# CERALIVE/ceracoder

Hardware: AMD Instinct MI355X
Metric: 1080p H.264 encoded frames/sec per GPU (higher is better)
Workload: dtype u8

## Files before the change

### ceracoder_amd/csrc/k_motion.hip

```cpp
#include "kernels_common.hpp"

#ifndef ME_MBS
#define ME_MBS 4
#endif
#define ME_WQ (ME_MBS + 2)
#define ME_ROWS 50
#define ME_STRIDE 53
#define ME_K 5

DEV unsigned long long qsad(unsigned lo, unsigned hi, unsigned cur, unsigned long long acc) {
    unsigned long long src = ((unsigned long long)hi << 32) | lo;
    return __builtin_amdgcn_qsad_pk_u16_u8(src, cur, acc);
}
DEV int mv_bits(int v) {
    int a = iabs(v);
    return a == 0 ? 1 : 7 + 2 * (31 - __clz(a));
}
DEV int med3(int a, int b, int c) {
    const int lo = a < b ? a : b, hi = a < b ? b : a;
    return c < lo ? lo : (c > hi ? hi : c);
}
struct fpred_t { int px, py, sx, sy; };
DEV fpred_t field_pred(const imv_t *__restrict__ f, int mbw, int mx, int my, bool top) {
    const bool avA = mx > 0, avB = top, avC = top && mx + 1 < mbw, avD = mx > 0 && top, hasC = avC || avD;
// ... 220 lines not shown
#pragma unroll
        for (int d = 0; d < ME_K; d++) { const uint2 v = ldg64(sf + (ME_K * g + d) * SURF_COLS); acc[d] = ((unsigned long long)v.y << 32) | v.x; }
        const unsigned best = select_min(acc, g, dxg, active, ctx->me_range, ctx->lambda, jpx, jpy, jsx, jsy);
        if (lane == 0) store_imv(&out[mbn], best, ctx->lambda, jpx, jpy, jsx, jsy);
    }
}

#define SP_GS 24
#define SP_PS 20
struct sp_lds {
    uint8_t G[23 * SP_GS];
    int16_t H1[18 * SP_GS];
    uint8_t b[19 * SP_PS];
    uint8_t h[18 * SP_GS];
    uint8_t j[18 * SP_PS];
    uint8_t pad[16];
};
typedef short sp_s2 __attribute__((ext_vector_type(2)));
DEV sp_s2 as_s2(unsigned v) { return __builtin_bit_cast(sp_s2, v); }
DEV unsigned as_u(sp_s2 v) { return __builtin_bit_cast(unsigned, v); }
DEV sp_s2 bytes_lo(unsigned w) { return as_s2(__builtin_amdgcn_perm(0u, w, 0x0c010c00u)); }
DEV sp_s2 bytes_hi(unsigned w) { return as_s2(__builtin_amdgcn_perm(0u, w, 0x0c030c02u)); }
DEV sp_s2 clip255_s2(sp_s2 v) { return __builtin_elementwise_min(__builtin_elementwise_max(v, (sp_s2)(0)), (sp_s2)(255)); }
DEV sp_s2 pair_s2(int a, int b) { return as_s2(__builtin_amdgcn_perm((unsigned)b, (unsigned)a, 0x05040100u)); }
DEV unsigned pack_s2(sp_s2 lo, sp_s2 hi) { return __builtin_amdgcn_perm(as_u(hi), as_u(lo), 0x06040200u); }
DEV unsigned clip_pack4(int a, int b, int c, int d) { return pack_s2(clip255_s2(pair_s2(a, b)), clip255_s2(pair_s2(c, d))); }
DEV int mvq_bits(int q) {
    unsigned k = q > 0 ? (unsigned)(2 * q - 1) : (unsigned)(-2 * q);
    return 2 * (31 - __clz((int)(k + 1))) + 1;
}
DEV unsigned lds4(const uint8_t *plane, int o) {
    const unsigned *w = (const unsigned *)(plane + (o & ~3));
    return __builtin_amdgcn_alignbyte(w[1], w[0], (unsigned)(o & 3));
}
DEV unsigned sp_sample4(const sp_lds *L, int X, int Y, int fx, int fy) {
#define SG(x, y) lds4(L->G, ((y) + 2) * SP_GS + (x) + 2)
#define SB(x, y) lds4(L->b, (y) * SP_PS + (x))
#define SH(x, y) lds4(L->h, (y) * SP_GS + (x) + 2)
#define SJ(x, y) lds4(L->j, (y) * SP_PS + (x))
    if (fy == 0) {
        if (fx == 0) return SG(X, Y);
        return fx == 2 ? SB(X, Y) : fx == 1 ? avg4(SG(X, Y), SB(X, Y)) : avg4(SG(X + 1, Y), SB(X, Y));
    }
    if (fx == 0) return fy == 2 ? SH(X, Y) : fy == 1 ? avg4(SG(X, Y), SH(X, Y)) : avg4(SG(X, Y + 1), SH(X, Y));
    if ((fx & 1) && (fy & 1)) return avg4(fy == 1 ? SB(X, Y) : SB(X, Y + 1), fx == 1 ? SH(X, Y) : SH(X + 1, Y));
    if (fx == 2 && fy == 2) return SJ(X, Y);
    if (fx == 2) return avg4(fy == 1 ? SB(X, Y) : SB(X, Y + 1), SJ(X, Y));
    return avg4(fx == 1 ? SH(X, Y) : SH(X + 1, Y), SJ(X, Y));
#undef SG
#undef SB
#undef SH
#undef SJ
}
DEV void sp_planes(sp_lds *L, const int lane) {
    if (lane < 54) {
        const int d = lane % 6, seg = lane / 6;
        sp_s2 lo[7], hi[7];
#pragma unroll
        for (int r = 0; r < 7; r++) {
            const unsigned w = *(const unsigned *)&L->G[(2 * seg + r) * SP_GS + 4 * d];
            lo[r] = bytes_lo(w); hi[r] = bytes_hi(w);
        }
#pragma unroll
        for (int t = 0; t < 2; t++) {
            const sp_s2 vl = (lo[t + 2] + lo[t + 3]) * (sp_s2)(20) - (lo[t + 1] + lo[t + 4]) * (sp_s2)(5) + (lo[t] + lo[t + 5]);
            const sp_s2 vh = (hi[t + 2] + hi[t + 3]) * (sp_s2)(20) - (hi[t + 1] + hi[t + 4]) * (sp_s2)(5) + (hi[t] + hi[t + 5]);
            const int R = 2 * seg + t;
            unsigned *o = (unsigned *)&L->H1[R * SP_GS + 4 * d];
            o[0] = as_u(vl); o[1] = as_u(vh);
            *(unsigned *)&L->h[R * SP_GS + 4 * d] = pack_s2(clip255_s2((vl + (sp_s2)(16)) >> (sp_s2)(5)), clip255_s2((vh + (sp_s2)(16)) >> (sp_s2)(5)));
        }
    }
#pragma unroll
    for (int it = 0; it < 2; it++) {
        const int i = lane + 64 * it;
        if (i < 19 * 5) {
            const int R = i / 5, g = i - R * 5;
            const unsigned *gw = (const unsigned *)&L->G[(R + 2) * SP_GS + 4 * g];
            const unsigned d0 = gw[0] ^ 0x80808080u, d1 = gw[1] ^ 0x80808080u, d2 = gw[2] ^ 0x80808080u;
            int o[4];
#pragma unroll
            for (int k = 0; k < 4; k++) {
                const unsigned w0 = k ? __builtin_amdgcn_alignbyte(d1, d0, (unsigned)k) : d0, w1 = k ? __builtin_amdgcn_alignbyte(d2, d1, (unsigned)k) : d1;
                const int v = __builtin_amdgcn_sdot4((int)w0, 0x1414FB01, __builtin_amdgcn_sdot4((int)w1, 0x000001FB, 4096, false), false);
                o[k] = (v + 16) >> 5;
            }
            *(unsigned *)&L->b[R * SP_PS + 4 * g] = clip_pack4(o[0], o[1], o[2], o[3]);
        }
    }
    WAVE_SYNC();
#pragma unroll
    for (int it = 0; it < 2; it++) {
        const int i = lane + 64 * it;
        if (i < 18 * 5) {
            const int R = i / 5, g = i - R * 5;
            const unsigned *hw = (const unsigned *)&L->H1[R * SP_GS + 4 * g];
            const unsigned p0 = hw[0], p1 = hw[1], p2 = hw[2], p3 = hw[3], p4 = hw[4];
            const unsigned q0 = __builtin_amdgcn_alignbyte(p1, p0, 2u), q1 = __builtin_amdgcn_alignbyte(p2, p1, 2u),
                           q2 = __builtin_amdgcn_alignbyte(p3, p2, 2u), q3 = __builtin_amdgcn_alignbyte(p4, p3, 2u);
            const sp_s2 ca = {1, -5}, cb = {20, 20}, cc = {-5, 1};
#define J3(a, b, c) __builtin_amdgcn_sdot2(as_s2(a), ca, __builtin_amdgcn_sdot2(as_s2(b), cb, __builtin_amdgcn_sdot2(as_s2(c), cc, 512, false), false), false)
            const int v0 = J3(p0, p1, p2), v1 = J3(q0, q1, q2), v2 = J3(p1, p2, p3), v3 = J3(q1, q2, q3);
#undef J3
            *(unsigned *)&L->j[R * SP_PS + 4 * g] = clip_pack4(v0 >> 10, v1 >> 10, v2 >> 10, v3 >> 10);
        }
    }
// ... 27 lines not shown
            L->G[r * SP_GS + c] = (uint8_t)ldg8(ref + (size_t)yy * stride + xx);
        }
    const int pr = lane >> 2, pc = (lane & 3) * 4;
    unsigned curw;
    {
        int sy = y0 + pr;
        sy = sy < ctx->vis_h ? sy : ctx->vis_h - 1;
        curw = ldg32(ctx->src_y + (size_t)sy * ctx->src_stride + x0 + pc);
    }
    WAVE_SYNC();
    sp_planes(L, lane);
    const int lambda = ctx->lambda;
    int bqx = info.mvx, bqy = info.mvy;
    unsigned best = info.cost;
#pragma unroll 1
    for (int step = 2; step >= 1; step--) {
        const int cqx = bqx, cqy = bqy;
        unsigned acc[4] = {0, 0, 0, 0};
#pragma unroll
        for (int c8 = 0; c8 < 8; c8++) {
            const int k = c8 < 4 ? c8 : c8 + 1;
            const int qx = cqx + (k % 3 - 1) * step, qy = cqy + (k / 3 - 1) * step;
            const int ox = qx - info.mvx, oy = qy - info.mvy;
            const int X = 1 + (ox >> 2) + pc, Y = 1 + (oy >> 2) + pr;
            const unsigned sad = __builtin_amdgcn_sad_u8(curw, sp_sample4(L, X, Y, ox & 3, oy & 3), 0u);
            acc[c8 >> 1] |= sad << (16 * (c8 & 1));
        }
#pragma unroll
        for (int q = 0; q < 4; q++) {
            acc[q] = (unsigned)wave64_sum((int)acc[q]);
        }
#pragma unroll
        for (int c8 = 0; c8 < 8; c8++) {
            const int k = c8 < 4 ? c8 : c8 + 1;
            const int qx = cqx + (k % 3 - 1) * step, qy = cqy + (k / 3 - 1) * step;
            const unsigned sad = (acc[c8 >> 1] >> (16 * (c8 & 1))) & 0xFFFFu;
            const unsigned cost = sad + (unsigned)(lambda * (mvq_bits(qx) + mvq_bits(qy)));
            if (cost < best) { best = cost; bqx = qx; bqy = qy; }
        }
    }
    if (lane == 0 && ok) {
        mb_info_t *mb = &ctx->mbi[mbn];
        stg32(&mb->mvx, ((unsigned)(uint16_t)bqx) | ((unsigned)(uint16_t)bqy << 16));
        stg32(&mb->cost, best);
    }
}

DEV int dec_score(unsigned M) { return dec_score_mask(M); }
DEV int row_or4(int v) {
    v |= __builtin_amdgcn_update_dpp(0, v, 0x128, 0xF, 0xF, false);
    v |= __builtin_amdgcn_update_dpp(0, v, 0x124, 0xF, 0xF, false);
    return v;
}
DEV unsigned ref_word4(const uint8_t *__restrict__ ref, int stride, int W, int H, int x, int y, bool inside) {
    if (inside) {
        const uint8_t *b = ref + (size_t)y * stride + (x & ~3);
        return __builtin_amdgcn_alignbyte(ldg32(b + 4), ldg32(b), (unsigned)(x & 3));
    }
    const uint8_t *r = ref + (size_t)clip3(0, H - 1, y) * stride;
    return pack4((int)ldg8(r + clip3(0, W - 1, x)), (int)ldg8(r + clip3(0, W - 1, x + 1)), (int)ldg8(r + clip3(0, W - 1, x + 2)), (int)ldg8(r + clip3(0, W - 1, x + 3)));
}
DEV void chroma_pred4(const frame_ctx_t *__restrict__ ctx, int lane, int x0, int y0, int W, int H, int mvx, int mvy, int *pd) {
    const int stride = ctx->stride;
    const int py = (lane >> 2) & 3, cby = (lane >> 4) & 1, c = (lane >> 1) & 1, cbx = lane & 1;
    const int cx0 = x0 >> 1, cy0 = y0 >> 1, cw = W >> 1, ch = H >> 1;
    const int cy = cby * 4 + py, cxb = cbx * 4;
    const int xi = mvx >> 3, yi = mvy >> 3, xf = mvx & 7, yf = mvy & 7;
    const uint8_t *__restrict__ rf = ctx->ref_uv;
    int A[5], B[5];
    if (cx0 + xi >= 0 && cx0 + xi + 9 <= cw && cy0 + yi >= 0 && cy0 + yi + 9 <= ch) {
        const int o = 2 * (cx0 + cxb + xi) + c, a = o & 3;
        const uint8_t *r0 = rf + (size_t)(cy0 + cy + yi) * stride + (o & ~3), *r1 = r0 + stride;
        const unsigned a0 = ldg32(r0), a1 = ldg32(r0 + 4), a2 = ldg32(r0 + 8), b0 = ldg32(r1), b1 = ldg32(r1 + 4), b2 = ldg32(r1 + 8);
        const unsigned sa0 = __builtin_amdgcn_alignbyte(a1, a0, (unsigned)a), sa1 = __builtin_amdgcn_alignbyte(a2, a1, (unsigned)a);
        const unsigned sb0 = __builtin_amdgcn_alignbyte(b1, b0, (unsigned)a), sb1 = __builtin_amdgcn_alignbyte(b2, b1, (unsigned)a);
        A[0] = byte_of(sa0, 0); A[1] = byte_of(sa0, 2); A[2] = byte_of(sa1, 0); A[3] = byte_of(sa1, 2); A[4] = (int)((a2 >> (8 * a)) & 255);
        B[0] = byte_of(sb0, 0); B[1] = byte_of(sb0, 2); B[2] = byte_of(sb1, 0); B[3] = byte_of(sb1, 2); B[4] = (int)((b2 >> (8 * a)) & 255);
    } else {
        const int ya = clip3(0, ch - 1, cy0 + cy + yi), yb = clip3(0, ch - 1, cy0 + cy + yi + 1);
#pragma unroll
        for (int i = 0; i < 5; i++) {
            const int xx = clip3(0, cw - 1, cx0 + cxb + i + xi);
            A[i] = (int)ldg8(rf + (size_t)ya * stride + 2 * xx + c);
            B[i] = (int)ldg8(rf + (size_t)yb * stride + 2 * xx + c);
        }
    }
    const int w00 = (8 - xf) * (8 - yf), w10 = xf * (8 - yf), w01 = (8 - xf) * yf, w11 = xf * yf;
#pragma unroll
    for (int i = 0; i < 4; i++) pd[i] = (w00 * A[i] + w10 * A[i + 1] + w01 * B[i] + w11 * B[i + 1] + 32) >> 6;
}
DEV unsigned pmb_luma_tq(const dev_tables *T, int lane, unsigned curw, unsigned pw, int qp, bool decimate, int *lev, int *x) {
    const int py = (lane >> 2) & 3, fy = ((py & 1) << 1) | (py >> 1);
    const col_bf cb = make_col_bf(py);
    const int kz0 = (int)((0xFEA9DB83C7426510ull >> (16 * fy)) & 0xFFFF);
    const qparams q = make_q(T, qp, false);
    const int mfe = py < 2 ? q.mf[0] : q.mf[2], mfo = py < 2 ? q.mf[2] : q.mf[1], ve = py < 2 ? q.v[0] : q.v[2], vo = py < 2 ? q.v[2] : q.v[1];
#pragma unroll
    for (int i = 0; i < 4; i++) x[i] = byte_of(curw, i) - byte_of(pw, i);
    fwd_rows4(x);
    unsigned m = 0, big = 0;
#pragma unroll
    for (int i = 0; i < 4; i++) {
        const int cf = fwd_col(x[i], cb);
        lev[i] = quant1(cf, (i & 1) ? mfo : mfe, q.f, q.qbits);
        m |= (lev[i] != 0 ? 1u : 0u) << ((kz0 >> (4 * i)) & 15);
        big |= (lev[i] > 1 || lev[i] < -1) ? 1u : 0u;
    }
    if (decimate) {
        const unsigned mm = (unsigned)row_or4((int)(m | (big << 16)));
        int s = (mm >> 16) ? 9 : dec_score(((mm & 0xFFFFu) << 1) | 1u);
        int s8 = s + quad_xor<1>(s);
        s8 += __shfl_xor(s8, 16, 64);
        int tot = s8 + quad_xor<2>(s8);
        tot += __shfl_xor(tot, 32, 64);
        if (s8 < 4 || tot < 6) { lev[0] = lev[1] = lev[2] = lev[3] = 0; }
    }
#pragma unroll
    for (int i = 0; i < 4; i++) x[i] = (lev[i] * ((i & 1) ? vo : ve)) << q.shift;
    const unsigned long long bal = __ballot((lev[0] | lev[1] | lev[2] | lev[3]) != 0);
    const unsigned long long t = bal | (bal >> 4) | (bal >> 8) | (bal >> 12);
    const int rb = lane & 15, rbx = blkx(rb) >> 2, rby = blky(rb) >> 2;
    return (unsigned)(__ballot(lane < 16 && ((t >> (16 * rby + rbx)) & 1)) & 0xFFFFull);
}
DEV unsigned pmb_satd(int lane, unsigned curw, unsigned pw) {
    const int py = (lane >> 2) & 3, s1 = py < 2 ? 1 : -1, s2 = (py & 1) ? -1 : 1;
    const int d0 = byte_of(curw, 0) - byte_of(pw, 0), d1 = byte_of(curw, 1) - byte_of(pw, 1), d2 = byte_of(curw, 2) - byte_of(pw, 2), d3 = byte_of(curw, 3) - byte_of(pw, 3);
    const int a = d0 + d3, b = d1 + d2, c = d1 - d2, e = d0 - d3;
    int t[4] = {a + b, e + c, a - b, e - c};
    int acc = 0;
#pragma unroll
    for (int i = 0; i < 4; i++) {
        const int u = mad24(t[i], s1, row_xor8(t[i]));
        const int w = mad24(u, s2, row_xor4(u));
        acc += iabs(w);
    }
    return (unsigned)wave64_sum(acc);
}
DEV unsigned pmb_sa8d(int lane, unsigned curw, unsigned pw) {
    const int s0 = (lane & 1) ? -1 : 1, s1 = (lane & 4) ? -1 : 1, s2 = (lane & 8) ? -1 : 1, s3 = (lane & 16) ? -1 : 1;
    const int d0 = byte_of(curw, 0) - byte_of(pw, 0), d1 = byte_of(curw, 1) - byte_of(pw, 1), d2 = byte_of(curw, 2) - byte_of(pw, 2), d3 = byte_of(curw, 3) - byte_of(pw, 3);
    const int a = d0 + d3, b = d1 + d2, c = d1 - d2, e = d0 - d3;
    int t[4] = {a + b, e + c, a - b, e - c};
    int acc = 0;
#pragma unroll
    for (int i = 0; i < 4; i++) {
        int u = mad24(t[i], s0, quad_xor<1>(t[i]));
        u = mad24(u, s1, row_xor4(u));
        u = mad24(u, s2, row_xor8(u));
        u = mad24(u, s3, __shfl_xor(u, 16, 64));
        acc += iabs(u);
    }
    return (unsigned)wave64_sum(acc);
}
DEV bool pmb_pick_t8(int lane, unsigned curw, unsigned pw) {
    const unsigned raw4 = pmb_satd(lane, curw, pw), raw8 = pmb_sa8d(lane, curw, pw);
    return __builtin_amdgcn_readfirstlane((int)(((raw8 + 2) >> 2) < (raw4 >> 1))) != 0;
}
template <bool SC1>
DEV void pmb_store_pred_only(const frame_ctx_t *__restrict__ ctx, int16_t *lv, int lane, int x0, int y0, unsigned pw, const int *pd) {
    const int stride = ctx->stride, pr = lane >> 2, pc = (lane & 3) * 4;
    stx32<SC1>(ctx->rec_y + (size_t)(y0 + pr) * stride + x0 + pc, pw);
    const int py = (lane >> 2) & 3, cby = (lane >> 4) & 1, c = (lane >> 1) & 1, cbx = lane & 1;
    const unsigned mine = pack4(pd[0], pd[1], pd[2], pd[3]), other = (unsigned)quad_xor<2>((int)mine);
    if (lane < 32 && c == 0) {
        uint2 out;
        out.x = __builtin_amdgcn_perm(other, mine, 0x05010400u);
        out.y = __builtin_amdgcn_perm(other, mine, 0x07030602u);
        stx64<SC1>(ctx->rec_uv + (size_t)((y0 >> 1) + cby * 4 + py) * stride + 2 * ((x0 >> 1) + cbx * 4), out);
    }
    if (lane < MB_LEVELS * 2 / 16) stg128(lv + 8 * lane, make_uint4(0, 0, 0, 0));
}

template <bool SC1>
DEV unsigned pmb_luma_t8(const frame_ctx_t *__restrict__ ctx, int *tile, int lane, unsigned curw, unsigned pw, int qp, int mbn, int x0, int y0) {
    const int pr = lane >> 2, pc = (lane & 3) * 4;
    {
        int *t = tile + ((pr >> 3) * 2 + (pc >> 3)) * 64 + (pr & 7) * 8 + (pc & 7);
#pragma unroll
        for (int i = 0; i < 4; i++) t[i] = byte_of(curw, i) - byte_of(pw, i);
    }
    WAVE_SYNC();
    const bool act = lane < 16;
    const int i8 = (lane >> 2) & 3, j = lane & 3;
    int *tb = tile + i8 * 64;
    const int m6 = qp % 6, k6 = qp / 6;
    int rs[2][8], cw[2][8];
    unsigned submask = 0;
    if (act) {
#pragma unroll
        for (int r = 0; r < 2; r++) {
// ... 81 lines not shown
        for (int i = 0; i < 4; i++) o[i] = clip255(byte_of(pw, i) + t[i]);
        stx32<SC1>(ctx->rec_y + (size_t)(y0 + pr) * ctx->stride + x0 + pc, pack4(o[0], o[1], o[2], o[3]));
    }
    return (unsigned)(__ballot(act && ((submask >> j) & 1u)) & 0xFFFFull);
}
DEV unsigned part_gsum(unsigned v) {
    v += (unsigned)quad_xor<1>((int)v);
    v += (unsigned)row_xor4((int)v);
    v += (unsigned)row_xor8((int)v);
    v += (unsigned)__shfl_xor((int)v, 16, 64);
    return v;
}
DEV unsigned part_total(unsigned g) { g += (unsigned)quad_xor<2>((int)g); return g + (unsigned)__shfl_xor((int)g, 32, 64); }
#ifdef PMB_PROF
#define PMB_NPH 11
#define PMB_MARK(k) do { const unsigned long long t1_ = __builtin_readcyclecounter(); ph_[k] = t1_ - t0_; t0_ = t1_; } while (0)
#define PMB_MARK0() unsigned long long ph_[PMB_NPH] = {0, 0, 0, 0, 0, 0, 0, 0, 0, 0, 0}; unsigned long long t0_ = __builtin_readcyclecounter()
#define PMB_FLUSH() do { if (lane == 0) for (int k_ = 0; k_ < PMB_NPH; k_++) stg32((unsigned *)ctx->dbrec + (size_t)mbn * 16 + k_, (unsigned)ph_[k_]); } while (0)
#else
#define PMB_MARK(k) ((void)0)
#define PMB_MARK0() ((void)0)
#define PMB_FLUSH() ((void)0)
#endif
struct pmb_pre_t { uint2 selfw; fpred_t fp; unsigned curw; uint2 sw; unsigned ds; uint4 dw; };
DEV pmb_pre_t pmb_preload(const frame_ctx_t *__restrict__ ctx, const int mbn, const int lane) {
    const int mbw = ctx->mbw, my = mbn / mbw, mx = mbn - my * mbw, x0 = mx * 16, y0 = my * 16;
    pmb_pre_t p;
    const imv_t *__restrict__ field = k_final_imv_dev(ctx);
    p.selfw = ldg64(field + mbn);
    {
        int sy = y0 + (lane >> 2);
        sy = sy < ctx->vis_h ? sy : ctx->vis_h - 1;
        p.curw = ldg32(ctx->src_y + (size_t)sy * ctx->src_stride + x0 + (lane & 3) * 4);
    }
    {
        const int cby = (lane >> 4) & 1, cbx = lane & 1;
        int sy = (y0 >> 1) + cby * 4 + ((lane >> 2) & 3);
        const int vh2 = ctx->vis_h >> 1;
        sy = sy < vh2 ? sy : vh2 - 1;
        p.sw = ldg64(ctx->src_uv + (size_t)sy * ctx->src_stride + 2 * ((x0 >> 1) + cbx * 4));
    }
    p.dw = ctx->intra_p ? ldg128(ctx->idec + (size_t)mbn * IDEC_BYTES + 16) : make_uint4(0, 0, 0, 0);
    p.fp = field_pred(field, mbw, mx, my, row_has_top(ctx, my));
    p.ds = (unsigned)*(const GAS uint16_t *)(ctx->surf + (size_t)mbn * SURF_U16 + ((p.fp.sy >> 2) + 16) * SURF_COLS + (p.fp.sx >> 2) + 16);
    return p;
}
DEV bool ir_ok(const frame_ctx_t *__restrict__ ctx, int mx, int mvx) {
    return mx >= ctx->ir_c0 || (16 * mx + 15 + (mvx >> 2) + ((mvx & 3) ? 3 : 0) <= ctx->ir_clean && 8 * mx + 7 + (mvx >> 3) + ((mvx & 7) ? 1 : 0) <= (ctx->ir_clean >> 1));
}
DEV int ir_max_whole(const frame_ctx_t *__restrict__ ctx, int mx) {
    const int kl = ctx->ir_clean - 16 * mx - 15, kc = 2 * ((ctx->ir_clean >> 1) - 8 * mx - 7);
    return 4 * (kl < kc ? kl : kc);
}
template <bool SC1>
DEV void pmb_store_intra(mb_info_t *mb, const uint4 dw, int qp, int lane) {
    if (lane == 0) {
        const bool i4 = ((dw.x >> 16) & 255u) != 0;
        mb_info_t m;
        m.mvx = 0; m.mvy = 0; m.mb_type = i4 ? 2 : 0; m.i16_mode = i4 ? 0 : (uint8_t)(dw.x & 255u); m.chroma_mode = (uint8_t)((dw.x >> 8) & 255u);
        m.qp = (uint8_t)qp; m.nzmask = 0; m.cost = dw.y;
        st_mbinfo_x<SC1>(mb, m);
    }
}
template <bool SC1, bool PART, int T8, bool IR>
DEV void pmb_mb(const frame_ctx_t *__restrict__ ctx, sp_lds *L, const int mbn, const int lane, const int refine, const pmb_pre_t &pre) {
    const int mbw = ctx->mbw, mbh = ctx->mbh, stride = ctx->stride, W = mbw * 16, H = mbh * 16, qp = mb_qp_dev(ctx, mbn), lambda = ctx->lambda;
    const int my = mbn / mbw, mx = mbn - my * mbw, x0 = mx * 16, y0 = my * 16;
    const dev_tables *T = &g_tab;
    PMB_MARK0();
    const uint2 selfw = pre.selfw;
    int imx = (int)(int16_t)(selfw.x & 0xFFFF);
    const int imy = (int)(int16_t)(selfw.x >> 16);
    const unsigned di = selfw.y & 0xFFFFu, ibits = selfw.y >> 16;
    const fpred_t fp = pre.fp;
    const int pr = lane >> 2, pc = (lane & 3) * 4;
    const int py = (lane >> 2) & 3;
    const unsigned curw = pre.curw;
    int sv[4];
    {
        const int c = (lane >> 1) & 1;
        const uint2 sw = pre.sw;
        const unsigned slo = c ? (sw.x >> 8) : sw.x, shi = c ? (sw.y >> 8) : sw.y;
        sv[0] = (int)(slo & 255); sv[1] = (int)((slo >> 16) & 255); sv[2] = (int)(shi & 255); sv[3] = (int)((shi >> 16) & 255);
    }
    int16_t *lv = ctx->levels + (size_t)mbn * MB_LEVELS;
    mb_info_t *mb = &ctx->mbi[mbn];
    if (IR && mx >= ctx->ir_c0 && mx < ctx->ir_c1) {
        pmb_store_intra<SC1>(mb, pre.dw, qp, lane);
        PMB_FLUSH();
        return;
    }
    {
        const unsigned ds = pre.ds;
        const bool skip_ok = !IR || ir_ok(ctx, mx, fp.sx);
        bool pass = ctx->drop_sad && ds < ctx->drop_sad && skip_ok;
        const bool worth = ds <= di + (unsigned)(lambda * SKIP_MARGIN_BITS) && skip_ok;
        PMB_MARK(0);
        if (pass || worth) {
            const int X = x0 + (fp.sx >> 2), Y = y0 + (fp.sy >> 2);
            const bool inside = X >= 0 && Y >= 0 && X + 16 <= W && Y + 16 <= H;
            const unsigned pw = ref_word4(ctx->ref_y, stride, W, H, X + pc, Y + pr, inside);
            int pd[4];
            chroma_pred4(ctx, lane, x0, y0, W, H, fp.sx, fp.sy, pd);
            if (!pass) {
                int lev[4], x[4];
                if (pmb_luma_tq(T, lane, curw, pw, qp, true, lev, x) == 0) {
                    unsigned nz_c = 0, dc_c = 0;
                    chroma_rows4(ctx, T, lv, x0 >> 1, y0 >> 1, lane, pd, sv, qp, false, false, nullptr, nz_c, dc_c, true, 0, SC1);
                    pass = (nz_c | dc_c) == 0;
                }
            }
            PMB_MARK(1);
            if (pass) {
                pmb_store_pred_only<SC1>(ctx, lv, lane, x0, y0, pw, pd);
                if (lane == 0) {
                    mb_info_t m;
                    m.mvx = (int16_t)fp.sx; m.mvy = (int16_t)fp.sy; m.mb_type = 1; m.i16_mode = 0; m.chroma_mode = 0; m.qp = (uint8_t)qp; m.nzmask = 0; m.cost = di;
                    st_mbinfo_x<SC1>(mb, m);
                }
                PMB_FLUSH();
                return;
            }
        }
    }
    if (IR && !ir_ok(ctx, mx, imx)) imx = ir_max_whole(ctx, mx);
    const int ix = x0 + (imx >> 2), iy = y0 + (imy >> 2);
    const uint8_t *__restrict__ ref = ctx->ref_y;
    if (ix - 3 >= 0 && iy - 3 >= 0 && ((ix - 3) & ~3) + 28 <= W && iy + 19 < H) {
        const int a = (ix - 3) & 3;
        const uint8_t *base = ref + (size_t)(iy - 3) * stride + ((ix - 3) & ~3);
        for (int i = lane; i < 23 * 6; i += 64) {
            const int r = i / 6, d = i - r * 6;
            const unsigned w0 = ldg32(base + (size_t)r * stride + 4 * d), w1 = ldg32(base + (size_t)r * stride + 4 * d + 4);
            *(unsigned *)&L->G[r * SP_GS + 4 * d] = __builtin_amdgcn_alignbyte(w1, w0, (unsigned)a);
        }
    } else
        for (int i = lane; i < 23 * 23; i += 64) {
            int r = i / 23, c = i - r * 23;
            int yy = clip3(0, H - 1, iy - 3 + r), xx = clip3(0, W - 1, ix - 3 + c);
            L->G[r * SP_GS + c] = (uint8_t)ldg8(ref + (size_t)yy * stride + xx);
        }
    WAVE_SYNC();
    PMB_MARK(2);
    int bqx = imx, bqy = imy;
    unsigned q0 = 0, qh[4] = {0, 0, 0, 0}, qq[4] = {0, 0, 0, 0};
    int hbx = imx, hby = imy;
    unsigned best;
    if (PART) {
        q0 = part_gsum(__builtin_amdgcn_sad_u8(curw, sp_sample4(L, 1 + pc, 1 + pr, 0, 0), 0u));
        best = part_total(q0) + (unsigned)(lambda * (mvq_bits(imx - fp.px) + mvq_bits(imy - fp.py)));
    } else
        best = (unsigned)wave64_sum((int)__builtin_amdgcn_sad_u8(curw, sp_sample4(L, 1 + pc, 1 + pr, 0, 0), 0u)) +
               (unsigned)(lambda * (mvq_bits(imx - fp.px) + mvq_bits(imy - fp.py)));
    PMB_MARK(3);
    if (refine) {
        sp_planes(L, lane);
        PMB_MARK(4);
        {
            const int cqx = bqx, cqy = bqy;
            unsigned acc[4] = {0, 0, 0, 0};
#pragma unroll
            for (int c8 = 0; c8 < 8; c8++) {
                const int k = c8 < 4 ? c8 : c8 + 1;
                const int qx = cqx + (k % 3 - 1) * 2, qy = cqy + (k / 3 - 1) * 2;
                const int ox = qx - imx, oy = qy - imy;
                const unsigned sad = __builtin_amdgcn_sad_u8(curw, sp_sample4(L, 1 + (ox >> 2) + pc, 1 + (oy >> 2) + pr, ox & 3, oy & 3), 0u);
                acc[c8 >> 1] |= sad << (16 * (c8 & 1));
            }
#pragma unroll
            for (int q = 0; q < 4; q++) {
                if (PART) { qh[q] = part_gsum(acc[q]); acc[q] = part_total(qh[q]); }
                else acc[q] = (unsigned)wave64_sum((int)acc[q]);
            }
#pragma unroll
            for (int c8 = 0; c8 < 8; c8++) {
                const int k = c8 < 4 ? c8 : c8 + 1;
                const int qx = cqx + (k % 3 - 1) * 2, qy = cqy + (k / 3 - 1) * 2;
                const unsigned sad = (acc[c8 >> 1] >> (16 * (c8 & 1))) & 0xFFFFu;
                const unsigned cost = sad + (unsigned)(lambda * (mvq_bits(qx - fp.px) + mvq_bits(qy - fp.py)));
                if (cost < best && (!IR || ir_ok(ctx, mx, qx))) { best = cost; bqx = qx; bqy = qy; }
            }
        }
        hbx = bqx; hby = bqy;
        PMB_MARK(5);
        {
            const int cqx = bqx, cqy = bqy;
            {
                const int ox = cqx - imx, oy = cqy - imy;
                best = (pmb_satd(lane, curw, sp_sample4(L, 1 + (ox >> 2) + pc, 1 + (oy >> 2) + pr, ox & 3, oy & 3)) >> 1) +
                       (unsigned)(lambda * (mvq_bits(cqx - fp.px) + mvq_bits(cqy - fp.py)));
            }
#pragma unroll 1
            for (int k = 0; k < 9; k++) {
                if (k == 4) continue;
                const int qx = cqx + (k % 3 - 1), qy = cqy + (k / 3 - 1);
                const int ox = qx - imx, oy = qy - imy;
                const unsigned cw = sp_sample4(L, 1 + (ox >> 2) + pc, 1 + (oy >> 2) + pr, ox & 3, oy & 3);
                if (PART) {
                    const int c8 = k < 4 ? k : k - 1;
                    const unsigned g = part_gsum(__builtin_amdgcn_sad_u8(curw, cw, 0u)) << (16 * (c8 & 1));
                    qq[0] |= (c8 >> 1) == 0 ? g : 0u; qq[1] |= (c8 >> 1) == 1 ? g : 0u; qq[2] |= (c8 >> 1) == 2 ? g : 0u; qq[3] |= (c8 >> 1) == 3 ? g : 0u;
                }
                const unsigned d = pmb_satd(lane, curw, cw) >> 1;
                const unsigned cost = d + (unsigned)(lambda * (mvq_bits(qx - fp.px) + mvq_bits(qy - fp.py)));
                if (cost < best && (!IR || ir_ok(ctx, mx, qx))) { best = cost; bqx = qx; bqy = qy; }
            }
        }
    }
    PMB_MARK(6);
    const int ox = bqx - imx, oy = bqy - imy;
    unsigned pw = sp_sample4(L, 1 + (ox >> 2) + pc, 1 + (oy >> 2) + pr, ox & 3, oy & 3);
    unsigned dsad = (unsigned)wave64_sum((int)__builtin_amdgcn_sad_u8(curw, pw, 0u));
    unsigned jinter = dsad + (unsigned)(lambda * (mvq_bits(bqx - fp.px) + mvq_bits(bqy - fp.py)));
    int shape = 0, lvx = bqx, lvy = bqy;
    if (PART && refine) {
        unsigned k8 = 0xFFFFFFFFu, k168 = 0xFFFFFFFFu, k816 = 0xFFFFFFFFu;
#pragma unroll 1
        for (int k = 0; k < 17; k++) {
            const int cx = k == 0 ? imx : k < 9 ? imx + (((k - 1 < 4 ? k - 1 : k) % 3) - 1) * 2 : hbx + (((k - 9 < 4 ? k - 9 : k - 8) % 3) - 1);
            const int cy = k == 0 ? imy : k < 9 ? imy + (((k - 1 < 4 ? k - 1 : k) / 3) - 1) * 2 : hby + (((k - 9 < 4 ? k - 9 : k - 8) / 3) - 1);
            const unsigned bits = (unsigned)(lambda * (mvq_bits(cx - fp.px) + mvq_bits(cy - fp.py)));
            const int c8 = k == 0 ? 0 : k < 9 ? k - 1 : k - 9;
            const unsigned pk = k == 0 ? q0 : k < 9 ? ((c8 >> 1) == 0 ? qh[0] : (c8 >> 1) == 1 ? qh[1] : (c8 >> 1) == 2 ? qh[2] : qh[3])
                                                    : ((c8 >> 1) == 0 ? qq[0] : (c8 >> 1) == 1 ? qq[1] : (c8 >> 1) == 2 ? qq[2] : qq[3]);
            const unsigned sq = k == 0 ? pk : (pk >> (16 * (c8 & 1))) & 0xFFFFu;
            const unsigned sh = sq + (unsigned)quad_xor<2>((int)sq);
            const unsigned sv_ = sq + (unsigned)__shfl_xor((int)sq, 32, 64);
            const unsigned a = ((sq + bits) << 5) | (unsigned)k, b = ((sh + bits) << 5) | (unsigned)k, c = ((sv_ + bits) << 5) | (unsigned)k;
            k8 = a < k8 ? a : k8; k168 = b < k168 ? b : k168; k816 = c < k816 ? c : k816;
        }
        const unsigned c8x8 = (k8 >> 5), c168 = (k168 >> 5), c816 = (k816 >> 5);
        unsigned t8 = c8x8 + (unsigned)quad_xor<2>((int)c8x8); t8 += (unsigned)__shfl_xor((int)t8, 32, 64);
        const unsigned t168 = c168 + (unsigned)__shfl_xor((int)c168, 32, 64);
        const unsigned t816 = c816 + (unsigned)quad_xor<2>((int)c816);
        unsigned jb = jinter + (unsigned)lambda;
        unsigned key = 0;
        const unsigned j1 = t168 + 3u * (unsigned)lambda, j2 = t816 + 3u * (unsigned)lambda, j3 = t8 + 9u * (unsigned)lambda;
        if (j1 < jb) { jb = j1; shape = 1; key = k168; }
        if (j2 < jb) { jb = j2; shape = 2; key = k816; }
        if (j3 < jb) { jb = j3; shape = 3; key = k8; }
        shape = __builtin_amdgcn_readfirstlane(shape);
        if (shape) {
            const int k = (int)(key & 31u);
            lvx = k == 0 ? imx : k < 9 ? imx + (((k - 1 < 4 ? k - 1 : k) % 3) - 1) * 2 : hbx + (((k - 9 < 4 ? k - 9 : k - 8) % 3) - 1);
            lvy = k == 0 ? imy : k < 9 ? imy + (((k - 1 < 4 ? k - 1 : k) / 3) - 1) * 2 : hby + (((k - 9 < 4 ? k - 9 : k - 8) / 3) - 1);
            const int px_ = lvx - imx, py_ = lvy - imy;
            pw = sp_sample4(L, 1 + (px_ >> 2) + pc, 1 + (py_ >> 2) + pr, px_ & 3, py_ & 3);
            dsad = (unsigned)wave64_sum((int)__builtin_amdgcn_sad_u8(curw, pw, 0u));
            jinter = jb - (unsigned)lambda;
        }
    }
    if (ctx->intra_p && di + (unsigned)lambda * ibits >= INTRA_GATE(lambda)) {
        const uint4 dw = pre.dw;
        const unsigned jintra = dw.z + (dw.z >> 3) + (unsigned)(lambda * 12);
        if (jintra < jinter) {
            pmb_store_intra<SC1>(mb, dw, qp, lane);
            PMB_FLUSH();
// ... 12 lines not shown
        slot = lane == 0 ? v1 : (shape == 3 && lane == 1) ? v2 : (shape == 3 && lane == 2) ? v3 : 0u;
        bqx = __builtin_amdgcn_readfirstlane(lvx); bqy = __builtin_amdgcn_readfirstlane(lvy);
    } else chroma_pred4(ctx, lane, x0, y0, W, H, bqx, bqy, pd);
    if (ctx->drop_sad && dsad < ctx->drop_sad) {
        pmb_store_pred_only<SC1>(ctx, lv, lane, x0, y0, pw, pd);
        if (PART && shape && lane < 8) stx32<SC1>(lv + L_LDC + 2 * lane, slot);
        if (lane == 0) {
            mb_info_t m;
            m.mvx = (int16_t)bqx; m.mvy = (int16_t)bqy; m.mb_type = 1; m.i16_mode = (uint8_t)shape; m.chroma_mode = 0; m.qp = (uint8_t)qp; m.nzmask = 0; m.cost = di;
            st_mbinfo_x<SC1>(mb, m);
        }
        PMB_FLUSH();
        return;
    }
    PMB_MARK(8);
    unsigned nz_luma;
    const bool t8 = T8 == 1 || (T8 == 2 && pmb_pick_t8(lane, curw, pw));
    if (t8) {
        nz_luma = pmb_luma_t8<SC1>(ctx, (int *)L, lane, curw, pw, qp, mbn, x0, y0);
    } else {
        const int fy = ((py & 1) << 1) | (py >> 1);
        const col_bf cb = make_col_bf(py);
        const int kz0 = (int)((0xFEA9DB83C7426510ull >> (16 * fy)) & 0xFFFF);
        int lev[4], x[4];
        nz_luma = pmb_luma_tq(T, lane, curw, pw, qp, true, lev, x);
        const int bx = lane & 3, by = lane >> 4, b = ((by >> 1) << 3) | ((bx >> 1) << 2) | ((by & 1) << 1) | (bx & 1);
#pragma unroll
        for (int i = 0; i < 4; i++) stg16(&lv[L_LUMA + b * 16 + ((kz0 >> (4 * i)) & 15)], lev[i]);
        inv_rows4(x);
        int o[4];
#pragma unroll
        for (int i = 0; i < 4; i++) o[i] = clip255(byte_of(pw, i) + ((inv_col(x[i], cb) + 32) >> 6));
        stx32<SC1>(ctx->rec_y + (size_t)(y0 + pr) * stride + x0 + pc, pack4(o[0], o[1], o[2], o[3]));
    }
    PMB_MARK(9);
    unsigned nz_c = 0, dc_c = 0;
    chroma_rows4(ctx, T, lv, x0 >> 1, y0 >> 1, lane, pd, sv, qp, false, true, nullptr, nz_c, dc_c, true, 0, SC1);
    PMB_MARK(10);
    if (lane == 0) {
        unsigned nzm = nz_luma | (nz_c << 16);
        if (dc_c & 1) nzm |= NZ_CBDC;
        if (dc_c & 2) nzm |= NZ_CRDC;
        if (t8 && nz_luma) nzm |= NZ_T8;
        mb_info_t m;
        m.mvx = (int16_t)bqx; m.mvy = (int16_t)bqy; m.mb_type = 1; m.i16_mode = (uint8_t)shape; m.chroma_mode = 0; m.qp = (uint8_t)qp; m.nzmask = nzm; m.cost = di;
        st_mbinfo_x<SC1>(mb, m);
    }
    if (PART && shape) { if (lane < 8) stx32<SC1>(lv + L_LDC + 2 * lane, slot); }
    else if (lane < 2) stg128(lv + L_LDC + 8 * lane, make_uint4(0, 0, 0, 0));
    PMB_FLUSH();
}

template <bool GATED, bool ROWS, bool PART, int T8, bool IR = false>
__global__ __launch_bounds__(256) void pmb_kernel(const frame_ctx_t cv, int mb0, int mb1, int refine, const unsigned *__restrict__ gate_done, unsigned ref_epoch, unsigned *err, unsigned *row_done) {
    const frame_ctx_t *__restrict__ ctx = &cv;
    __shared__ __attribute__((aligned(16))) sp_lds LD[4];
    const int lane = threadIdx.x & 63, wave = __builtin_amdgcn_readfirstlane(threadIdx.x >> 6);
    const int mbn = mb0 + 4 * (int)blockIdx.x + wave;
    if (mb0 == 0 && blockIdx.x == 0) tl_first(ctx, 2);
    pmb_pre_t pre;
    if (mbn < mb1) pre = pmb_preload(ctx, mbn, lane);
    if (GATED) {
        if (wave == 0) {
            const int mbw = ctx->mbw, mbh = ctx->mbh;
            const int first = mb0 + 4 * (int)blockIdx.x, last = first + 3 < mb1 ? first + 3 : mb1 - 1;
            int r_lo = first / mbw - 2, r_hi = last / mbw + 2;
            r_lo = r_lo > 0 ? r_lo : 0;
            r_hi = r_hi < mbh ? r_hi : mbh - 1;
            const uint2 *flags = (const uint2 *)(gate_done + DB_DONE_STRIDE * (blockIdx.x & (DB_DONE_COPIES - 1)));
            const int b_hi = r_hi / MI355_BAND_ROWS;
#ifdef DBG_OLD_GATE
            int spins = 0, b = b_hi;
#else
            int spins = 0, b = r_lo / MI355_BAND_ROWS;
#endif
            for (;;) {
                const uint2 f = ld64_sc1(flags + b);
                if (f.x == ref_epoch && f.y == ref_epoch) { if (++b > b_hi) break; continue; }
#ifndef PMB_POLL_SLEEP
#define PMB_POLL_SLEEP 64
#endif
                __builtin_amdgcn_s_sleep(PMB_POLL_SLEEP);
                if (++spins > DB_SPIN_MAX) { st_sc1(err, 3u); break; }
                if ((spins & 255) == 0 && ld_sc1(err)) break;
            }
            __builtin_amdgcn_fence(__ATOMIC_ACQUIRE, "agent");
        }
        __syncthreads();
        tl_last(ctx, 3);
    }
    if (mbn >= mb1) return;
    pmb_mb<ROWS, PART, T8, IR>(ctx, &LD[wave], mbn, lane, refine, pre);
    if (ROWS) {
        asm volatile("s_waitcnt vmcnt(0)" ::: "memory");
        if (lane == 0) __hip_atomic_fetch_add(row_done + (mbn / ctx->mbw) * MI355_PROG_STRIDE, 1u, __ATOMIC_RELAXED, __HIP_MEMORY_SCOPE_AGENT);
    }
    tl_last(ctx, 4);
}

__global__ __launch_bounds__(256) void copy_luma_kernel(const frame_ctx_t cv) {
    const frame_ctx_t *__restrict__ ctx = &cv;
    const int W = ctx->mbw * 16, H = ctx->mbh * 16, per_row = W / 16;
    const int i = blockIdx.x * 256 + threadIdx.x;
    if (i >= per_row * H) return;
    const int y = i / per_row, x = (i - y * per_row) * 16;
    const int sy = y < ctx->vis_h ? y : ctx->vis_h - 1;
    stg128(ctx->psrc_out + (size_t)y * ctx->stride + x, ldg128(ctx->src_y + (size_t)sy * ctx->src_stride + x));
// ... 79 lines not shown
```

Measured before the change: 7474.

## Overlap skip-probe loads with search-window fetch and batch quarter-pel SATD refinement

```diff
diff --git a/ceracoder_amd/csrc/k_motion.hip b/ceracoder_amd/csrc/k_motion.hip
--- a/ceracoder_amd/csrc/k_motion.hip
+++ b/ceracoder_amd/csrc/k_motion.hip
@@ -296,6 +296,18 @@
 #undef SH
 #undef SJ
 }
+DEV int sp_plane_off(int p, int x, int y) {
+    constexpr unsigned long long bases = (unsigned long long)(offsetof(sp_lds, G) + 2 * SP_GS + 2) | (unsigned long long)offsetof(sp_lds, b) << 16 |
+                                         (unsigned long long)(offsetof(sp_lds, h) + 2) << 32 | (unsigned long long)offsetof(sp_lds, j) << 48;
+    static_assert(sizeof(sp_lds) < 65536, "a plane's offset fits 16 bits");
+    return (int)((bases >> (16 * p)) & 0xFFFFu) + y * (SP_GS - (SP_GS - SP_PS) * (p & 1)) + x;
+}
+DEV unsigned sp_sample4_flat(const sp_lds *L, int X, int Y, int fx, int fy) {
+    const int f = 4 * fy + fx;
+    const int pa = (int)((0x54BA5410u >> (2 * f)) & 3u), pb = (int)((0xBAFEBA54u >> (2 * f)) & 3u);
+    const int adx = (0x0808 >> f) & 1, ady = (0xF000 >> f) & 1, bdx = (0x8080 >> f) & 1;
+    return avg4(lds4((const uint8_t *)L, sp_plane_off(pa, X + adx, Y + ady)), lds4((const uint8_t *)L, sp_plane_off(pb, X + bdx, Y)));
+}
 DEV void sp_planes(sp_lds *L, const int lane) {
     if (lane < 54) {
         const int d = lane % 6, seg = lane / 6;
@@ -429,42 +441,63 @@
     v |= __builtin_amdgcn_update_dpp(0, v, 0x124, 0xF, 0xF, false);
     return v;
 }
-DEV unsigned ref_word4(const uint8_t *__restrict__ ref, int stride, int W, int H, int x, int y, bool inside) {
+struct ref_raw_t { unsigned a, b, c, d; };
+DEV ref_raw_t ref_word4_load(const uint8_t *__restrict__ ref, int stride, int W, int H, int x, int y, bool inside) {
+    ref_raw_t w = {0, 0, 0, 0};
     if (inside) {
         const uint8_t *b = ref + (size_t)y * stride + (x & ~3);
-        return __builtin_amdgcn_alignbyte(ldg32(b + 4), ldg32(b), (unsigned)(x & 3));
-    }
-    const uint8_t *r = ref + (size_t)clip3(0, H - 1, y) * stride;
-    return pack4((int)ldg8(r + clip3(0, W - 1, x)), (int)ldg8(r + clip3(0, W - 1, x + 1)), (int)ldg8(r + clip3(0, W - 1, x + 2)), (int)ldg8(r + clip3(0, W - 1, x + 3)));
-}
-DEV void chroma_pred4(const frame_ctx_t *__restrict__ ctx, int lane, int x0, int y0, int W, int H, int mvx, int mvy, int *pd) {
+        w.a = ldg32(b); w.b = ldg32(b + 4);
+    } else {
+        const uint8_t *r = ref + (size_t)clip3(0, H - 1, y) * stride;
+        w.a = ldg8(r + clip3(0, W - 1, x)); w.b = ldg8(r + clip3(0, W - 1, x + 1)); w.c = ldg8(r + clip3(0, W - 1, x + 2)); w.d = ldg8(r + clip3(0, W - 1, x + 3));
+    }
+    return w;
+}
+DEV unsigned ref_word4_word(const ref_raw_t w, int x, bool inside) {
+    return inside ? __builtin_amdgcn_alignbyte(w.b, w.a, (unsigned)(x & 3)) : pack4((int)w.a, (int)w.b, (int)w.c, (int)w.d);
+}
+struct chroma_raw_t { unsigned a0, a1, a2, a3, a4, b0, b1, b2, b3, b4; bool inside; };
+DEV chroma_raw_t chroma_pred4_load(const frame_ctx_t *__restrict__ ctx, int lane, int x0, int y0, int W, int H, int mvx, int mvy) {
     const int stride = ctx->stride;
     const int py = (lane >> 2) & 3, cby = (lane >> 4) & 1, c = (lane >> 1) & 1, cbx = lane & 1;
     const int cx0 = x0 >> 1, cy0 = y0 >> 1, cw = W >> 1, ch = H >> 1;
     const int cy = cby * 4 + py, cxb = cbx * 4;
-    const int xi = mvx >> 3, yi = mvy >> 3, xf = mvx & 7, yf = mvy & 7;
+    const int xi = mvx >> 3, yi = mvy >> 3;
     const uint8_t *__restrict__ rf = ctx->ref_uv;
+    chroma_raw_t w = {0, 0, 0, 0, 0, 0, 0, 0, 0, 0, false};
+    w.inside = cx0 + xi >= 0 && cx0 + xi + 9 <= cw && cy0 + yi >= 0 && cy0 + yi + 9 <= ch;
+    if (w.inside) {
+        const int o = 2 * (cx0 + cxb + xi) + c;
+        const uint8_t *r0 = rf + (size_t)(cy0 + cy + yi) * stride + (o & ~3), *r1 = r0 + stride;
+        w.a0 = ldg32(r0); w.a1 = ldg32(r0 + 4); w.a2 = ldg32(r0 + 8); w.b0 = ldg32(r1); w.b1 = ldg32(r1 + 4); w.b2 = ldg32(r1 + 8);
+    } else {
+        const uint8_t *ra = rf + (size_t)clip3(0, ch - 1, cy0 + cy + yi) * stride + c, *rb = rf + (size_t)clip3(0, ch - 1, cy0 + cy + yi + 1) * stride + c;
+        const int xb = cx0 + cxb + xi;
+        const int o0 = 2 * clip3(0, cw - 1, xb), o1 = 2 * clip3(0, cw - 1, xb + 1), o2 = 2 * clip3(0, cw - 1, xb + 2), o3 = 2 * clip3(0, cw - 1, xb + 3), o4 = 2 * clip3(0, cw - 1, xb + 4);
+        w.a0 = ldg8(ra + o0); w.a1 = ldg8(ra + o1); w.a2 = ldg8(ra + o2); w.a3 = ldg8(ra + o3); w.a4 = ldg8(ra + o4);
+        w.b0 = ldg8(rb + o0); w.b1 = ldg8(rb + o1); w.b2 = ldg8(rb + o2); w.b3 = ldg8(rb + o3); w.b4 = ldg8(rb + o4);
+    }
+    return w;
+}
+DEV void chroma_pred4_finish(int lane, int x0, int mvx, int mvy, const chroma_raw_t w, int *pd) {
+    const int xf = mvx & 7, yf = mvy & 7;
     int A[5], B[5];
-    if (cx0 + xi >= 0 && cx0 + xi + 9 <= cw && cy0 + yi >= 0 && cy0 + yi + 9 <= ch) {
-        const int o = 2 * (cx0 + cxb + xi) + c, a = o & 3;
-        const uint8_t *r0 = rf + (size_t)(cy0 + cy + yi) * stride + (o & ~3), *r1 = r0 + stride;
-        const unsigned a0 = ldg32(r0), a1 = ldg32(r0 + 4), a2 = ldg32(r0 + 8), b0 = ldg32(r1), b1 = ldg32(r1 + 4), b2 = ldg32(r1 + 8);
-        const unsigned sa0 = __builtin_amdgcn_alignbyte(a1, a0, (unsigned)a), sa1 = __builtin_amdgcn_alignbyte(a2, a1, (unsigned)a);
-        const unsigned sb0 = __builtin_amdgcn_alignbyte(b1, b0, (unsigned)a), sb1 = __builtin_amdgcn_alignbyte(b2, b1, (unsigned)a);
-        A[0] = byte_of(sa0, 0); A[1] = byte_of(sa0, 2); A[2] = byte_of(sa1, 0); A[3] = byte_of(sa1, 2); A[4] = (int)((a2 >> (8 * a)) & 255);
-        B[0] = byte_of(sb0, 0); B[1] = byte_of(sb0, 2); B[2] = byte_of(sb1, 0); B[3] = byte_of(sb1, 2); B[4] = (int)((b2 >> (8 * a)) & 255);
+    if (w.inside) {
+        const int a = (2 * ((x0 >> 1) + (lane & 1) * 4 + (mvx >> 3)) + ((lane >> 1) & 1)) & 3;
+        const unsigned sa0 = __builtin_amdgcn_alignbyte(w.a1, w.a0, (unsigned)a), sa1 = __builtin_amdgcn_alignbyte(w.a2, w.a1, (unsigned)a);
+        const unsigned sb0 = __builtin_amdgcn_alignbyte(w.b1, w.b0, (unsigned)a), sb1 = __builtin_amdgcn_alignbyte(w.b2, w.b1, (unsigned)a);
+        A[0] = byte_of(sa0, 0); A[1] = byte_of(sa0, 2); A[2] = byte_of(sa1, 0); A[3] = byte_of(sa1, 2); A[4] = (int)((w.a2 >> (8 * a)) & 255);
+        B[0] = byte_of(sb0, 0); B[1] = byte_of(sb0, 2); B[2] = byte_of(sb1, 0); B[3] = byte_of(sb1, 2); B[4] = (int)((w.b2 >> (8 * a)) & 255);
     } else {
-        const int ya = clip3(0, ch - 1, cy0 + cy + yi), yb = clip3(0, ch - 1, cy0 + cy + yi + 1);
-#pragma unroll
-        for (int i = 0; i < 5; i++) {
-            const int xx = clip3(0, cw - 1, cx0 + cxb + i + xi);
-            A[i] = (int)ldg8(rf + (size_t)ya * stride + 2 * xx + c);
-            B[i] = (int)ldg8(rf + (size_t)yb * stride + 2 * xx + c);
-        }
+        A[0] = (int)w.a0; A[1] = (int)w.a1; A[2] = (int)w.a2; A[3] = (int)w.a3; A[4] = (int)w.a4;
+        B[0] = (int)w.b0; B[1] = (int)w.b1; B[2] = (int)w.b2; B[3] = (int)w.b3; B[4] = (int)w.b4;
     }
     const int w00 = (8 - xf) * (8 - yf), w10 = xf * (8 - yf), w01 = (8 - xf) * yf, w11 = xf * yf;
 #pragma unroll
     for (int i = 0; i < 4; i++) pd[i] = (w00 * A[i] + w10 * A[i + 1] + w01 * B[i] + w11 * B[i + 1] + 32) >> 6;
+}
+DEV void chroma_pred4(const frame_ctx_t *__restrict__ ctx, int lane, int x0, int y0, int W, int H, int mvx, int mvy, int *pd) {
+    chroma_pred4_finish(lane, x0, mvx, mvy, chroma_pred4_load(ctx, lane, x0, y0, W, H, mvx, mvy), pd);
 }
 DEV unsigned pmb_luma_tq(const dev_tables *T, int lane, unsigned curw, unsigned pw, int qp, bool decimate, int *lev, int *x) {
     const int py = (lane >> 2) & 3, fy = ((py & 1) << 1) | (py >> 1);
@@ -499,7 +532,7 @@
     const int rb = lane & 15, rbx = blkx(rb) >> 2, rby = blky(rb) >> 2;
     return (unsigned)(__ballot(lane < 16 && ((t >> (16 * rby + rbx)) & 1)) & 0xFFFFull);
 }
-DEV unsigned pmb_satd(int lane, unsigned curw, unsigned pw) {
+DEV unsigned pmb_satd_lane(int lane, unsigned curw, unsigned pw) {
     const int py = (lane >> 2) & 3, s1 = py < 2 ? 1 : -1, s2 = (py & 1) ? -1 : 1;
     const int d0 = byte_of(curw, 0) - byte_of(pw, 0), d1 = byte_of(curw, 1) - byte_of(pw, 1), d2 = byte_of(curw, 2) - byte_of(pw, 2), d3 = byte_of(curw, 3) - byte_of(pw, 3);
     const int a = d0 + d3, b = d1 + d2, c = d1 - d2, e = d0 - d3;
@@ -511,8 +544,9 @@
         const int w = mad24(u, s2, row_xor4(u));
         acc += iabs(w);
     }
-    return (unsigned)wave64_sum(acc);
-}
+    return (unsigned)acc;
+}
+DEV unsigned pmb_satd(int lane, unsigned curw, unsigned pw) { return (unsigned)wave64_sum((int)pmb_satd_lane(lane, curw, pw)); }
 DEV unsigned pmb_sa8d(int lane, unsigned curw, unsigned pw) {
     const int s0 = (lane & 1) ? -1 : 1, s1 = (lane & 4) ? -1 : 1, s2 = (lane & 8) ? -1 : 1, s3 = (lane & 16) ? -1 : 1;
     const int d0 = byte_of(curw, 0) - byte_of(pw, 0), d1 = byte_of(curw, 1) - byte_of(pw, 1), d2 = byte_of(curw, 2) - byte_of(pw, 2), d3 = byte_of(curw, 3) - byte_of(pw, 3);
@@ -700,6 +734,35 @@
     const int kl = ctx->ir_clean - 16 * mx - 15, kc = 2 * ((ctx->ir_clean >> 1) - 8 * mx - 7);
     return 4 * (kl < kc ? kl : kc);
 }
+DEV void pmb_window_to_lds(const uint8_t *__restrict__ ref, sp_lds *L, int lane, int ix, int iy, int W, int H, int stride) {
+    if (ix - 3 >= 0 && iy - 3 >= 0 && ((ix - 3) & ~3) + 28 <= W && iy + 19 < H) {
+        const int a = (ix - 3) & 3;
+        const uint8_t *base = ref + (size_t)(iy - 3) * stride + ((ix - 3) & ~3);
+        unsigned w0[3], w1[3];
+#pragma unroll
+        for (int t = 0; t < 3; t++) {
+            const int i = lane + 64 * t < 23 * 6 ? lane + 64 * t : 23 * 6 - 1, r = i / 6, d = i - r * 6;
+            w0[t] = ldg32(base + (size_t)r * stride + 4 * d); w1[t] = ldg32(base + (size_t)r * stride + 4 * d + 4);
+        }
+#pragma unroll
+        for (int t = 0; t < 3; t++) {
+            const int i = lane + 64 * t, r = i / 6, d = i - r * 6;
+            if (i < 23 * 6) *(unsigned *)&L->G[r * SP_GS + 4 * d] = __builtin_amdgcn_alignbyte(w1[t], w0[t], (unsigned)a);
+        }
+    } else {
+        unsigned v[9];
+#pragma unroll
+        for (int t = 0; t < 9; t++) {
+            const int i = lane + 64 * t < 23 * 23 ? lane + 64 * t : 23 * 23 - 1, r = i / 23, c = i - r * 23;
+            v[t] = ldg8(ref + (size_t)clip3(0, H - 1, iy - 3 + r) * stride + clip3(0, W - 1, ix - 3 + c));
+        }
+#pragma unroll
+        for (int t = 0; t < 9; t++) {
+            const int i = lane + 64 * t, r = i / 23, c = i - r * 23;
+            if (i < 23 * 23) L->G[r * SP_GS + c] = (uint8_t)v[t];
+        }
+    }
+}
 template <bool SC1>
 DEV void pmb_store_intra(mb_info_t *mb, const uint4 dw, int qp, int lane) {
     if (lane == 0) {
@@ -738,18 +801,27 @@
         PMB_FLUSH();
         return;
     }
+    if (IR && !ir_ok(ctx, mx, imx)) imx = ir_max_whole(ctx, mx);
     {
         const unsigned ds = pre.ds;
         const bool skip_ok = !IR || ir_ok(ctx, mx, fp.sx);
         bool pass = ctx->drop_sad && ds < ctx->drop_sad && skip_ok;
         const bool worth = ds <= di + (unsigned)(lambda * SKIP_MARGIN_BITS) && skip_ok;
         PMB_MARK(0);
-        if (pass || worth) {
-            const int X = x0 + (fp.sx >> 2), Y = y0 + (fp.sy >> 2);
-            const bool inside = X >= 0 && Y >= 0 && X + 16 <= W && Y + 16 <= H;
-            const unsigned pw = ref_word4(ctx->ref_y, stride, W, H, X + pc, Y + pr, inside);
+        const bool probe = pass || worth;
+        const int X = x0 + (fp.sx >> 2), Y = y0 + (fp.sy >> 2);
+        const bool inside = X >= 0 && Y >= 0 && X + 16 <= W && Y + 16 <= H;
+        ref_raw_t rawy = {0, 0, 0, 0};
+        chroma_raw_t rawc = {0, 0, 0, 0, 0, 0, 0, 0, 0, 0, false};
+        if (probe) {
+            rawy = ref_word4_load(ctx->ref_y, stride, W, H, X + pc, Y + pr, inside);
+            rawc = chroma_pred4_load(ctx, lane, x0, y0, W, H, fp.sx, fp.sy);
+        }
+        if (!pass) pmb_window_to_lds(ctx->ref_y, L, lane, x0 + (imx >> 2), y0 + (imy >> 2), W, H, stride);
+        if (probe) {
+            const unsigned pw = ref_word4_word(rawy, X + pc, inside);
             int pd[4];
-            chroma_pred4(ctx, lane, x0, y0, W, H, fp.sx, fp.sy, pd);
+            chroma_pred4_finish(lane, x0, fp.sx, fp.sy, rawc, pd);
             if (!pass) {
                 int lev[4], x[4];
                 if (pmb_luma_tq(T, lane, curw, pw, qp, true, lev, x) == 0) {
@@ -771,23 +843,6 @@
             }
         }
     }
-    if (IR && !ir_ok(ctx, mx, imx)) imx = ir_max_whole(ctx, mx);
-    const int ix = x0 + (imx >> 2), iy = y0 + (imy >> 2);
-    const uint8_t *__restrict__ ref = ctx->ref_y;
-    if (ix - 3 >= 0 && iy - 3 >= 0 && ((ix - 3) & ~3) + 28 <= W && iy + 19 < H) {
-        const int a = (ix - 3) & 3;
-        const uint8_t *base = ref + (size_t)(iy - 3) * stride + ((ix - 3) & ~3);
-        for (int i = lane; i < 23 * 6; i += 64) {
-            const int r = i / 6, d = i - r * 6;
-            const unsigned w0 = ldg32(base + (size_t)r * stride + 4 * d), w1 = ldg32(base + (size_t)r * stride + 4 * d + 4);
-            *(unsigned *)&L->G[r * SP_GS + 4 * d] = __builtin_amdgcn_alignbyte(w1, w0, (unsigned)a);
-        }
-    } else
-        for (int i = lane; i < 23 * 23; i += 64) {
-            int r = i / 23, c = i - r * 23;
-            int yy = clip3(0, H - 1, iy - 3 + r), xx = clip3(0, W - 1, ix - 3 + c);
-            L->G[r * SP_GS + c] = (uint8_t)ldg8(ref + (size_t)yy * stride + xx);
-        }
     WAVE_SYNC();
     PMB_MARK(2);
     int bqx = imx, bqy = imy;
@@ -831,7 +886,7 @@
         }
         hbx = bqx; hby = bqy;
         PMB_MARK(5);
-        {
+        if (PART) {
             const int cqx = bqx, cqy = bqy;
             {
                 const int ox = cqx - imx, oy = cqy - imy;
@@ -844,13 +899,37 @@
                 const int qx = cqx + (k % 3 - 1), qy = cqy + (k / 3 - 1);
                 const int ox = qx - imx, oy = qy - imy;
                 const unsigned cw = sp_sample4(L, 1 + (ox >> 2) + pc, 1 + (oy >> 2) + pr, ox & 3, oy & 3);
-                if (PART) {
-                    const int c8 = k < 4 ? k : k - 1;
-                    const unsigned g = part_gsum(__builtin_amdgcn_sad_u8(curw, cw, 0u)) << (16 * (c8 & 1));
-                    qq[0] |= (c8 >> 1) == 0 ? g : 0u; qq[1] |= (c8 >> 1) == 1 ? g : 0u; qq[2] |= (c8 >> 1) == 2 ? g : 0u; qq[3] |= (c8 >> 1) == 3 ? g : 0u;
-                }
+                const int c8 = k < 4 ? k : k - 1;
+                const unsigned g = part_gsum(__builtin_amdgcn_sad_u8(curw, cw, 0u)) << (16 * (c8 & 1));
+                qq[0] |= (c8 >> 1) == 0 ? g : 0u; qq[1] |= (c8 >> 1) == 1 ? g : 0u; qq[2] |= (c8 >> 1) == 2 ? g : 0u; qq[3] |= (c8 >> 1) == 3 ? g : 0u;
                 const unsigned d = pmb_satd(lane, curw, cw) >> 1;
                 const unsigned cost = d + (unsigned)(lambda * (mvq_bits(qx - fp.px) + mvq_bits(qy - fp.py)));
+                if (cost < best && (!IR || ir_ok(ctx, mx, qx))) { best = cost; bqx = qx; bqy = qy; }
+            }
+        } else {
+            const int cqx = bqx, cqy = bqy;
+            const int cox = __builtin_amdgcn_readfirstlane(cqx - imx), coy = __builtin_amdgcn_readfirstlane(cqy - imy);
+            unsigned sat[9];
+#pragma unroll
+            for (int k = 0; k < 9; k++) {
+                const int ox = cox + (k % 3 - 1), oy = coy + (k / 3 - 1);
+                sat[k] = sp_sample4_flat(L, 1 + (ox >> 2) + pc, 1 + (oy >> 2) + pr, ox & 3, oy & 3);
+                if (k == 2 || k == 5) __builtin_amdgcn_sched_barrier(0);
+            }
+#pragma unroll
+            for (int k = 0; k < 9; k++) {
+                __builtin_amdgcn_sched_barrier(0);
+                sat[k] = pmb_satd_lane(lane, curw, sat[k]);
+            }
+            __builtin_amdgcn_sched_barrier(0);
+#pragma unroll
+            for (int k = 0; k < 9; k++) sat[k] = (unsigned)wave64_sum((int)sat[k]);
+            best = (sat[4] >> 1) + (unsigned)(lambda * (mvq_bits(cqx - fp.px) + mvq_bits(cqy - fp.py)));
+#pragma unroll
+            for (int k = 0; k < 9; k++) {
+                if (k == 4) continue;
+                const int qx = cqx + (k % 3 - 1), qy = cqy + (k / 3 - 1);
+                const unsigned cost = (sat[k] >> 1) + (unsigned)(lambda * (mvq_bits(qx - fp.px) + mvq_bits(qy - fp.py)));
                 if (cost < best && (!IR || ir_ok(ctx, mx, qx))) { best = cost; bqx = qx; bqy = qy; }
             }
         }
@@ -969,7 +1048,7 @@
 }
 
 template <bool GATED, bool ROWS, bool PART, int T8, bool IR = false>
-__global__ __launch_bounds__(256) void pmb_kernel(const frame_ctx_t cv, int mb0, int mb1, int refine, const unsigned *__restrict__ gate_done, unsigned ref_epoch, unsigned *err, unsigned *row_done) {
+__global__ __launch_bounds__(256, T8 ? 4 : 8) void pmb_kernel(const frame_ctx_t cv, int mb0, int mb1, int refine, const unsigned *__restrict__ gate_done, unsigned ref_epoch, unsigned *err, unsigned *row_done) {
     const frame_ctx_t *__restrict__ ctx = &cv;
     __shared__ __attribute__((aligned(16))) sp_lds LD[4];
     const int lane = threadIdx.x & 63, wave = __builtin_amdgcn_readfirstlane(threadIdx.x >> 6);
```

After: 7355. 0.984x the previous value.
